# soosiey/gnn-formation-control

Hardware: NVIDIA B200
Metric: agent-graphs/sec fwd+bwd (GSO build+K-hop filter) (higher is better)
Workload: dtype f32

## Files before the change

### gnn-formation-control_b200/csrc/gfc_tc5_wide.cu

```cuda
#include <cuda.h>
#include <cudaTypedefs.h>
#include <type_traits>
#include "gfc_common.cuh"
#include "gfc_tc5.cuh"
#include "gfc_tc5_wide.cuh"
#include <string.h>

namespace gfc {
using tc5::make_desc;
using tc5::store_chunk_f16;

constexpr int kWideTop = 14;
constexpr int kPackHeader = 256;

template <int CIN, int COUT, int NP>
struct WideLayout {
  static constexpr int ROWS = 128;
  static constexpr int CS = CIN / 2;
  static constexpr int CPT = CS / 2;
  static constexpr int NCH = CS / 8;
  static constexpr int PW = ROWS * 16;
  static constexpr int PLANE = NCH * PW;
  static constexpr int SLAB = NP * PLANE;
  static constexpr int STAGE = COUT * 32 * NP;
  static constexpr int KSTEPS = CS / 16;
  static constexpr int PHASE = KSTEPS * STAGE;
  static constexpr int NSTAGE = 2;
  static constexpr int OFF_W = 0;
  static constexpr int OFF_RING = OFF_W + 4 * SLAB;
  static constexpr int OFF_STAGE = (OFF_RING + NSTAGE * PHASE + 1023) / 1024 * 1024;
  static constexpr int OFF_BIAS = OFF_STAGE + ROWS * 128;
  static constexpr int OFF_SP = OFF_BIAS + COUT * 4;
  static constexpr int OFF_DEG = OFF_SP + 2 * ROWS * 8;
  static constexpr int OFF_TAB = OFF_DEG + 2 * 2 * ROWS * 4;
  static constexpr int OFF_MAX = OFF_TAB + 3 * 128 * 4;
  static constexpr int OFF_BAR = OFF_MAX + 64;
  static constexpr int NBAR = 2 * NSTAGE + 2 + 2 + 2 + 1 + 2 + 2 + 2;
  static constexpr int BYTES = OFF_BAR + NBAR * 8 + 16;
  static constexpr int TM_OUT = 0;
  static constexpr int TM_HOP = 2 * COUT;
  static constexpr int TM_P = 2 * COUT + 2 * CS;
  static constexpr int TM_USED = 2 * COUT + 2 * CS + 128;
  static constexpr int TM_COLS = TM_USED <= 32 ? 32 : TM_USED <= 64 ? 64 : TM_USED <= 128 ? 128 : TM_USED <= 256 ? 256 : 512;
  static_assert(CIN % 32 == 0 && CIN >= 32 && CIN <= 128, "CIN in {32,64,96,128}");
  static_assert(COUT % 32 == 0 && COUT >= 32 && COUT <= 128, "COUT multiple of 32, <= 128");
  static_assert(CPT % 8 == 0, "whole chunks per worker thread");
  static_assert(BYTES <= 227 * 1024, "shared memory");
};
__device__ __forceinline__ int row_degree(const int* sdeg, int pbuf, int row) {
  const int* p = sdeg + pbuf * 2 * 128 + row;
  return p[0] + p[128];
}
__device__ __forceinline__ int row_degree4(const int* sdeg, int pbuf, int row) {
  const int* p = sdeg + pbuf * 4 * 128 + row;
  return p[0] + p[128] + p[256] + p[384];
}

constexpr int kWideThreads = 576;
constexpr int kGroupWarps = 8;
int g_wide_flush_every = 3;
int g_wide_no_prefetch = 0;

static __device__ __noinline__ bool wide_adjacent_exact(float ax, float ay, float bx, float by, double thr) {
  return sqdist64(ax, ay, bx, by) <= thr;
}

__device__ __forceinline__ uint32_t adjacency8(const float2* __restrict__ sp, float2 me, int pr, int c0, int c_lo,
                                               int c_hi, int rows_used, double thr, float thr_lo, float thr_hi) {
  const int lo = max(c_lo, c0) - c0, hi = min(min(c_hi, rows_used), c0 + 8) - c0;
  if (hi <= lo || pr >= rows_used) return 0u;
  uint32_t valid = ((1u << hi) - 1u) & ~((1u << lo) - 1u);
  if ((unsigned)(pr - c0) < 8u) valid &= ~(1u << (pr - c0));
  uint32_t in = 0, out = 0;
#pragma unroll
  for (int i = 0; i < 8; ++i) {
    const float2 o = sp[c0 + i];
    const float dx = me.x - o.x, dy = me.y - o.y;
    const float sv = fmaf(dx, dx, dy * dy);
    in |= (sv < thr_lo ? 1u : 0u) << i;
    out |= (sv > thr_hi ? 1u : 0u) << i;
  }
  uint32_t bits = in & valid;
  uint32_t band = valid & ~in & ~out;
  while (band) {
    const int i = __ffs(band) - 1;
    band &= band - 1;
    const float2 o = sp[c0 + i];
    if (wide_adjacent_exact(me.x, me.y, o.x, o.y, thr)) bits |= 1u << i;
  }
  return bits;
}
__device__ __forceinline__ uint32_t dense8(const float* __restrict__ Sg, int N, int transpose, int nr, int pr, int c0,
                                           int c_lo, int c_hi, int rows_used) {
  const int lo = max(c_lo, c0) - c0, hi = min(min(c_hi, rows_used), c0 + 8) - c0;
  if (hi <= lo || pr >= rows_used) return 0u;
  float v[8];
#pragma unroll
  for (int i = 0; i < 8; ++i) {
    const int m = c0 + i - c_lo;
    const bool ok = i >= lo && i < hi;
    const float* p = transpose ? Sg + (size_t)(ok ? m : 0) * N + nr : Sg + (size_t)nr * N + (ok ? m : 0);
    v[i] = ok ? __ldg(p) : 0.f;
  }
  uint32_t bits = 0;
#pragma unroll
  for (int i = 0; i < 8; ++i) bits |= (v[i] != 0.f ? 1u : 0u) << i;
  return bits;
}
__device__ __forceinline__ uint32_t p_word(uint32_t bits, int lo, uint32_t pv) {
  return ((bits >> lo) & 1u) * pv + ((bits >> (lo + 1)) & 1u) * (pv << 16);
}

__device__ __forceinline__ float ldg_f32(const float* p, bool pred) {
  float v;
  asm volatile(
      "{\n\t.reg .pred q;\n\t"
      "setp.ne.b32 q, %2, 0;\n\t"
      "mov.f32 %0, 0f00000000;\n\t"
      "@q ld.global.nc.f32 %0, [%1];\n\t}"
      : "=f"(v)
      : "l"(p), "r"((int)pred));
  return v;
}
__device__ __forceinline__ size_t wide_mask_word(int tile, int gw, int s, int lane) {
  return (((size_t)tile * 8 + gw) * 2 + s) * 32 + lane;
}
__device__ __forceinline__ size_t wide_fmask_word(int tile, int gw, int pcw, int lane) {
  return (((size_t)tile * 8 + gw) * 2 + pcw) * 32 + lane;
}
__device__ __forceinline__ size_t wide_fmask_locate(int tile, int row, int c, int F, int* shift) {
  const int hc = F >> 1, half = c >= hc ? 1 : 0, cc = c - half * hc;
  *shift = cc & 31;
  return wide_fmask_word(tile, half * 4 + (((row >> 5) + 2) & 3), cc >> 5, row & 31);
}
__device__ __forceinline__ uint32_t ldg_u32(const uint32_t* p, bool pred) {
  uint32_t v;
  asm volatile(
      "{\n\t.reg .pred q;\n\t"
      "setp.ne.b32 q, %2, 0;\n\t"
      "mov.b32 %0, 0;\n\t"
      "@q ld.global.nc.b32 %0, [%1];\n\t}"
      : "=r"(v)
      : "l"(p), "r"((int)pred));
  return v;
}
__device__ __forceinline__ float4 ldg_f32x4(const float* p, bool pred) {
  float4 v;
  asm volatile(
      "{\n\t.reg .pred q;\n\t"
      "setp.ne.b32 q, %5, 0;\n\t"
      "mov.f32 %0, 0f00000000;\n\tmov.f32 %1, 0f00000000;\n\tmov.f32 %2, 0f00000000;\n\tmov.f32 %3, 0f00000000;\n\t"
      "@q ld.global.nc.v4.f32 {%0,%1,%2,%3}, [%4];\n\t}"
      : "=f"(v.x), "=f"(v.y), "=f"(v.z), "=f"(v.w)
      : "l"(p), "r"((int)pred));
  return v;
}

__device__ __forceinline__ void red_add_f32(float* p, float v) {
  asm volatile("red.global.add.f32 [%0], %1;" ::"l"(p), "f"(v) : "memory");
}
__device__ __forceinline__ float ldg_cg(const float* p) {
  float v;
  asm volatile("ld.global.cg.f32 %0, [%1];" : "=f"(v) : "l"(p) : "memory");
  return v;
}
__device__ __forceinline__ void group_b_bar() { asm volatile("bar.sync 2, 256;" ::: "memory"); }
__device__ __forceinline__ void group_a_bar() { asm volatile("bar.sync 3, 256;" ::: "memory"); }

struct WideMaps { CUtensorMap m[2]; };

__device__ __forceinline__ float act_fast(float v, float neg, bool use_min) {
  const float t = v * neg;
  return use_min ? fminf(v, t) : fmaxf(v, t);
}

__device__ __forceinline__ void fill_degree_tables(float* tab, int tid, int nthreads) {
  for (int d = tid; d < 128; d += nthreads) {
    const float fd = (float)d;
    tab[d] = d ? 1.f / sqrtf(fd) : 1.f;
    tab[128 + d] = d ? 1.f / fd : 0.f;
    tab[256 + d] = d ? sqrtf(fd) : 1.f;
  }
}

template <int CIN, int COUT, int MODE, int NP>
__global__ void __launch_bounds__(kWideThreads, 1)
tc5_wide_kernel(const __grid_constant__ WideArgs w, const __grid_constant__ WideMaps maps) {
  using L = WideLayout<CIN, COUT, NP>;
  extern __shared__ __align__(128) unsigned char wsmem[];
  unsigned char* Wb = wsmem + L::OFF_W;
  unsigned char* Rb = wsmem + L::OFF_RING;
  float2* sp_all = reinterpret_cast<float2*>(wsmem + L::OFF_SP);
  int* sdeg = reinterpret_cast<int*>(wsmem + L::OFF_DEG);
  float* dtab = reinterpret_cast<float*>(wsmem + L::OFF_TAB);
  uint32_t* smax = reinterpret_cast<uint32_t*>(wsmem + L::OFF_MAX);
  unsigned char* stage_out = wsmem + L::OFF_STAGE;
  float* sbias = reinterpret_cast<float*>(wsmem + L::OFF_BIAS);
  uint64_t* bars = reinterpret_cast<uint64_t*>(wsmem + L::OFF_BAR);
  uint64_t* h_full = bars;
  uint64_t* h_empty = bars + L::NSTAGE;
  uint64_t* w_ready = bars + 2 * L::NSTAGE;
  uint64_t* hop_done = w_ready + 2;
  uint64_t* w0_free = hop_done + 2;
  uint64_t* p_ready = w0_free + 2;
  uint64_t* out_full = p_ready + 1;
  uint64_t* out_free = out_full + 2;
  uint64_t* w0_ready = out_free + 2;
  uint32_t* tmem_ptr = reinterpret_cast<uint32_t*>(w0_ready + 2);

  const int tid = threadIdx.x, lane = tid & 31, warp = tid >> 5;
  const int N = w.N, K = w.K;
  const bool norm = w.g.norm != 0;
  const int tiles_per_cta = (w.ntiles + (int)gridDim.x - 1) / (int)gridDim.x;
  const int t_begin = min(w.ntiles, (int)blockIdx.x * tiles_per_cta);
  const int t_end = min(w.ntiles, t_begin + tiles_per_cta);

  for (int i = tid; i < COUT; i += kWideThreads) sbias[i] = (MODE != 1 && w.bias) ? __ldg(w.bias + i) : 0.f;
  fill_degree_tables(dtab, tid, kWideThreads);
  if (tid == 0) {
    for (int i = 0; i < L::NSTAGE; ++i) { tc5::mbar_init(&h_full[i], 1); tc5::mbar_init(&h_empty[i], 1); }
    for (int i = 0; i < 2; ++i) {
      tc5::mbar_init(&w_ready[i], kGroupWarps);
      tc5::mbar_init(&w0_ready[i], kGroupWarps);
      tc5::mbar_init(&hop_done[i], 1);
      tc5::mbar_init(&w0_free[i], 1);
      tc5::mbar_init(&out_full[i], 1);
      tc5::mbar_init(&out_free[i], kGroupWarps);
    }
    tc5::mbar_init(p_ready, kGroupWarps);
    tc5::fence_mbar_init();
  }
  if (warp == 1) tc5::tmem_alloc(tmem_ptr, L::TM_COLS);
  tc5::fence_proxy_async();
  tc5::fence_before_sync();
  __syncthreads();
  tc5::fence_after_sync();
  const uint32_t tmem = *tmem_ptr;

  if (warp == 0) {
    if (tc5::elect_one()) {
      constexpr uint32_t kIdescTap = tc5::idesc_f16(128, COUT, 0, 0);
      constexpr uint32_t kIdescHop = tc5::idesc_f16(128, L::CS, 0, 1);
      const uint32_t w_addr = tc5::smem_u32(Wb), r_addr = tc5::smem_u32(Rb);
      uint32_t par_wr = 0, par_w0 = 0, par_of = 0, par_pr = 0, par_hf = 0;
      int st = 0;
      const int hop_ksteps = (w.gpc * N + 15) >> 4;
      int it = 0;
      int nstamp = 0;
      const bool dbg = w.dbg != nullptr && blockIdx.x == 0;
#ifdef GFC_WIDE_TIMELINE
#define GFC_WSTAMP(tag) do { if (dbg && nstamp < 2000) { w.dbg[2 * nstamp] = clock64(); w.dbg[2 * nstamp + 1] = (tag); ++nstamp; } } while (0)
#else
#define GFC_WSTAMP(tag) do { (void)dbg; (void)nstamp; } while (0)
#endif
      for (int tile = t_begin; tile < t_end; ++tile, ++it) {
        const int ob = it & 1;
        GFC_WSTAMP(1);
        if (K > 1) { tc5::mbar_wait(p_ready, par_pr); par_pr ^= 1; }
        GFC_WSTAMP(3);
        const uint32_t d_out = tmem + L::TM_OUT + ob * COUT;
#pragma unroll 1
        for (int ph = 0; ph < 2 * K; ++ph) {
          const int k = ph >> 1, s = ph & 1;
          GFC_WSTAMP(100 + ph);
          if (k == 0) { tc5::mbar_wait(&w0_ready[s], (par_w0 >> s) & 1); par_w0 ^= 1u << s; }
          else { tc5::mbar_wait(&w_ready[s], (par_wr >> s) & 1); par_wr ^= 1u << s; }
          tc5::fence_after_sync();
          GFC_WSTAMP(200 + ph);
          const uint32_t ws = w_addr + (2 * s + ((it * K + k) & 1)) * L::SLAB;
          if (k + 1 < K) {
            const uint32_t d_hop = tmem + L::TM_HOP + s * L::CS;
            uint32_t pa = tmem + L::TM_P + ob * 64;
            uint64_t bd = make_desc(ws, 128, L::PW);
            uint32_t acc = 0;
#pragma unroll 1
            for (int j = 0; j < hop_ksteps; ++j) {
              tc5::mma_bf16_ts(d_hop, pa, bd, kIdescHop, acc);
              if (NP == 2) tc5::mma_bf16_ts(d_hop, pa, bd + (L::PLANE >> 4), kIdescHop, 1u);
              acc = 1;
              pa += 8; bd += 256 >> 4;
            }
            tc5::mma_commit(&hop_done[s]);
          }
          if (ph == 0 && it >= 2) { tc5::mbar_wait(&out_free[ob], (par_of >> ob) & 1); par_of ^= 1u << ob; }
          tc5::mbar_wait(&h_full[st], (par_hf >> st) & 1); par_hf ^= 1u << st;
          tc5::fence_after_sync();
          {
            uint64_t a0 = make_desc(ws, L::PW, 128);
            uint64_t b0 = make_desc(r_addr + st * L::PHASE, COUT * 16, 128);
#pragma unroll
            for (int i = 0; i < L::KSTEPS; ++i) {
              tc5::mma_bf16_ss(d_out, a0, b0, kIdescTap, (ph == 0 && i == 0) ? 0u : 1u);
              if (NP == 2) {
                tc5::mma_bf16_ss(d_out, a0, b0 + ((COUT * 32) >> 4), kIdescTap, 1u);
                tc5::mma_bf16_ss(d_out, a0 + (L::PLANE >> 4), b0, kIdescTap, 1u);
              }
              a0 += (2 * L::PW) >> 4; b0 += L::STAGE >> 4;
            }
          }
          tc5::mma_commit(&h_empty[st]);
          st ^= 1;
          if (k == K - 2) tc5::mma_commit(&w0_free[s]);
          GFC_WSTAMP(300 + ph);
        }
        tc5::mma_commit(&out_full[ob]);
      }
#undef GFC_WSTAMP
    }
    __syncwarp();
  } else if (warp == 1) {
    if (tc5::elect_one()) {
      int st = 0;
// ... 281 lines not shown
          asm volatile("prefetch.global.L2 [%0];" ::"l"(yb + off));
      }
      if (tile + 1 < t_end) {
        const int nb = min(w.gpc, w.B - (b0 + w.gpc)) * N * CIN * 4;
        const char* db = reinterpret_cast<const char*>(w.in + (size_t)(b0 + w.gpc) * N * CIN);
        for (int off = wt * 128; off < nb; off += 32 * kGroupWarps * 128)
          asm volatile("prefetch.global.L2 [%0];" ::"l"(db + off));
      }
#pragma unroll 1
      for (int i0 = wt; i0 < n4; i0 += 8 * 32 * kGroupWarps) {
        float4 v[8];
#pragma unroll
        for (int u = 0; u < 8; ++u) {
          const int i = i0 + u * 32 * kGroupWarps;
          v[u] = ldg_f32x4(reinterpret_cast<const float*>(p + (i < n4 ? i : 0)), i < n4);
        }
#pragma unroll
        for (int u = 0; u < 8; ++u)
          m = fmaxf(fmaxf(m, fmaxf(fabsf(v[u].x), fabsf(v[u].y))), fmaxf(fabsf(v[u].z), fabsf(v[u].w)));
      }
      if (MODE == 1 && w.act == GFC_ACT_LEAKY_RELU && w.slope > 1.f) m *= w.slope;
      return m;
    };
    auto epilogue = [&](int tile, int ob, float inv) {
      const int b0 = tile * w.gpc;
      tc5::mbar_wait_suspend(&out_full[ob], (par_ofl >> ob) & 1); par_ofl ^= 1u << ob;
      tc5::fence_after_sync();
      GFC_KSTAMP(500);
      uint32_t fmw = 0;
      static_assert((COUT / 32) % 2 == 0, "two 16-channel pieces per mask word");
#pragma unroll 1
      for (int pc = 0; pc < COUT / 32; ++pc) {
        const int col = half * (COUT / 2) + pc * 16;
        uint32_t v[16];
        tc5::tmem_ld16(tm_lane + L::TM_OUT + ob * COUT + col, v);
        tc5::tmem_ld_wait();
        if constexpr (MODE != 1) {
          float4 o[4];
#pragma unroll
          for (int i4 = 0; i4 < 4; ++i4) {
            const float4 bb = *reinterpret_cast<const float4*>(sbias + col + i4 * 4);
            o[i4].x = act_fast(fmaf(__uint_as_float(v[i4 * 4 + 0]), inv, bb.x), act_neg, act_min);
            o[i4].y = act_fast(fmaf(__uint_as_float(v[i4 * 4 + 1]), inv, bb.y), act_neg, act_min);
            o[i4].z = act_fast(fmaf(__uint_as_float(v[i4 * 4 + 2]), inv, bb.z), act_neg, act_min);
            o[i4].w = act_fast(fmaf(__uint_as_float(v[i4 * 4 + 3]), inv, bb.w), act_neg, act_min);
          }
          if (w.fmask_out) {
            uint32_t b16 = 0;
#pragma unroll
            for (int i4 = 0; i4 < 4; ++i4)
              b16 |= ((o[i4].x > 0.f ? 1u : 0u) | (o[i4].y > 0.f ? 2u : 0u) | (o[i4].z > 0.f ? 4u : 0u) |
                      (o[i4].w > 0.f ? 8u : 0u)) << (4 * i4);
            if (r >= min(w.gpc, w.B - b0) * N) b16 = 0;
            fmw |= b16 << ((pc & 1) * 16);
            if (pc & 1) { w.fmask_out[wide_fmask_word(tile, gw, pc >> 1, lane)] = fmw; fmw = 0; }
          }
          if (lane == 0) tc5::tma_store_wait_read();
          __syncwarp();
          unsigned char* srow = slot_out + lane * 64;
          const int sw = (lane >> 1) & 3;
#pragma unroll
          for (int i4 = 0; i4 < 4; ++i4) *reinterpret_cast<float4*>(srow + ((i4 ^ sw) << 4)) = o[i4];
          tc5::fence_proxy_async();
          __syncwarp();
          if (lane == 0 && hq > 0) {
            tc5::tma_store_2d(my_map, slot_out, col, b0 * N + q * 32);
            tc5::tma_store_commit();
          }
        } else {
          const int rows_used = min(w.gpc, w.B - b0) * N;
          if (r < rows_used) {
            float* dst = w.out + ((size_t)(b0 + jr) * COUT + col) * N + nr;
#pragma unroll
            for (int i = 0; i < 16; ++i) dst[(size_t)i * N] = __uint_as_float(v[i]) * inv;
          }
        }
      }
      tc5::fence_before_sync();
      __syncwarp();
      if (lane == 0) tc5::mbar_arrive(&out_free[ob]);
      GFC_KSTAMP(501);
    };

    int next = t_begin, itn = 0;
    int epi_tile = -1, epi_ob = 0;
    while (true) {
      const bool has_next = next < t_end;
      if (!has_next && epi_tile < 0) break;
      if (has_next) {
        const int pbuf = itn & 1;
        group_b_bar();
        const float m = tile_max(next);
        const uint32_t mw = __reduce_max_sync(0xffffffffu, __float_as_uint(m));
        if (lane == 0) smax[gw] = mw;
        group_b_bar();
        uint32_t mt = smax[0];
#pragma unroll
        for (int i = 1; i < kGroupWarps; ++i) mt = max(mt, smax[i]);
        if (w.amax && wt == 0) atomicMax(reinterpret_cast<unsigned int*>(w.amax) + (MODE == 1 ? 1 : 0), mt);
        if (MODE == 0 && w.mark_stats && w.amax && wt == 0 && blockIdx.x == 0 && itn == 0) w.amax[3] = 1.f;
        scale_next = tc5::pow2_scale(mt, kWideTop, &inv_next);
        rowf_next = 1.f;
        if (norm && K > 1) {
          tc5::mbar_wait_suspend(p_ready, par_pb); par_pb ^= 1;
          tc5::fence_after_sync();
        }
        if (norm) {
          const int d = row_degree(sdeg, pbuf, r);
          rowf_next = dtab[d];
          inv_next *= dtab[256 + d];
        }
        inv_next *= inv_th;
        GFC_KSTAMP(401);
#pragma unroll 1
        for (int s = 0; s < 2; ++s) {
          load_slab(next, s);
          if (itn >= 1 && K >= 2) { tc5::mbar_wait_suspend(&w0_free[s], (par_w0 >> s) & 1); par_w0 ^= 1u << s; }
          GFC_KSTAMP(410 + s);
          store_slab(pbuf, Wb + (2 * s + ((itn * K) & 1)) * L::SLAB);
          tc5::fence_proxy_async();
          tc5::fence_before_sync();
          __syncwarp();
          if (lane == 0) tc5::mbar_arrive(&w0_ready[s]);
          GFC_KSTAMP(420 + s);
        }
      }
      if (epi_tile >= 0) { epilogue(epi_tile, epi_ob, inv_prev); epi_tile = -1; }
      if (has_next) { epi_tile = next; epi_ob = itn & 1; inv_prev = inv_next; ++next; ++itn; }
    }
    if (MODE != 1 && lane == 0) tc5::tma_store_wait_all();
#undef GFC_KSTAMP
  }
  tc5::fence_before_sync();
  __syncthreads();
  if (warp == 1) tc5::tmem_dealloc(tmem, L::TM_COLS);
}

template <int G, int F, int FH, int NP>
struct DhLayout {
  static constexpr int ROWS = 128;
  static constexpr int NFH = F / FH;
  static constexpr int CPT = FH / 4;
  static constexpr int NCH = FH / 8;
  static constexpr int PW = ROWS * 16;
  static constexpr int PLANE = NCH * PW;
  static constexpr int VBUF = NP * PLANE;
  static constexpr int P_BYTES = (ROWS / 8) * PW;
  static constexpr int OFF_V = 0;
  static constexpr int OFF_P = OFF_V + 3 * VBUF;
  static constexpr int OFF_SP = OFF_P + 2 * P_BYTES;
  static constexpr int OFF_DEG = OFF_SP + 2 * ROWS * 8;
  static constexpr int OFF_TAB = OFF_DEG + 2 * 4 * ROWS * 4;
  static constexpr int OFF_DB = OFF_TAB + 3 * 128 * 4;
  static constexpr int OFF_BAR = OFF_DB + FH * 4;
  static constexpr int NBAR = 7;
  static constexpr int BYTES_MIN = OFF_BAR + NBAR * 8 + 16;
  static constexpr int BYTES = BYTES_MIN < 120 * 1024 ? 120 * 1024 : BYTES_MIN;
  static constexpr int TM_X = 0;
  static constexpr int TM_ACC = NP * 64;
  static_assert(FH % 32 == 0 && F % FH == 0 && CPT % 8 == 0, "feature slice");
  static_assert(G == 128 || G == 64 || G == 32, "G");
  static_assert(BYTES <= 227 * 1024, "shared memory");
};

template <int G, int F, int FH, int NP, bool NV4>
__global__ void __launch_bounds__(kWideThreads, 1)
tc5_wide_dh_kernel(const __grid_constant__ WideDhArgs w) {
  using L = DhLayout<G, F, FH, NP>;
  extern __shared__ __align__(128) unsigned char wsmem[];
  unsigned char* Vb = wsmem + L::OFF_V;
  unsigned char* Pb = wsmem + L::OFF_P;
  float2* sp_all = reinterpret_cast<float2*>(wsmem + L::OFF_SP);
  int* sdeg = reinterpret_cast<int*>(wsmem + L::OFF_DEG);
  float* dtab = reinterpret_cast<float*>(wsmem + L::OFF_TAB);
  float* dbs = reinterpret_cast<float*>(wsmem + L::OFF_DB);
  uint64_t* bars = reinterpret_cast<uint64_t*>(wsmem + L::OFF_BAR);
  uint64_t* v_ready = bars;
  uint64_t* hop_done = bars + 1;
  uint64_t* item_done = bars + 2;
  uint64_t* p_ready = bars + 3;
  uint64_t* x_ready = bars + 4;
  uint64_t* v0_ready = bars + 5;
  uint64_t* v0_free = bars + 6;
  uint32_t* tmem_ptr = reinterpret_cast<uint32_t*>(bars + 7);

  const int tid = threadIdx.x, lane = tid & 31, warp = tid >> 5;
  const int N = w.N, K = w.K;
  const bool norm = w.g.norm != 0;
  const int fh = blockIdx.x % L::NFH, part = blockIdx.x / L::NFH, nparts = gridDim.x / L::NFH;
  const int TM_HOP = L::TM_ACC + K * FH;
  const bool merged = NP == 2 && (K + 2) * FH <= 384;
  const int tiles_per_part = (w.ntiles + nparts - 1) / nparts;
  const int t_begin = min(w.ntiles, part * tiles_per_part);
  const int t_end = min(w.ntiles, t_begin + tiles_per_part);

  for (int i = tid; i < 2 * L::P_BYTES / 16; i += kWideThreads) reinterpret_cast<uint4*>(Pb)[i] = make_uint4(0, 0, 0, 0);
  for (int i = tid; i < FH; i += kWideThreads) dbs[i] = 0.f;
  fill_degree_tables(dtab, tid, kWideThreads);
  if (tid == 0) {
    tc5::mbar_init(v_ready, kGroupWarps);
    tc5::mbar_init(hop_done, 1);
    tc5::mbar_init(item_done, 1);
    tc5::mbar_init(p_ready, kGroupWarps);
    tc5::mbar_init(x_ready, kGroupWarps);
    tc5::mbar_init(v0_ready, kGroupWarps);
    tc5::mbar_init(v0_free, 1);
    tc5::fence_mbar_init();
  }
  if (warp == 1) tc5::tmem_alloc(tmem_ptr, 512);
  tc5::fence_proxy_async();
  tc5::fence_before_sync();
  __syncthreads();
  tc5::fence_after_sync();
  const uint32_t tmem = *tmem_ptr;

  auto publish = [&](uint64_t* bar) {
    tc5::fence_proxy_async();
    tc5::fence_before_sync();
    __syncwarp();
    if (lane == 0) tc5::mbar_arrive(bar);
  };

  if (warp == 0) {
    if (tc5::elect_one()) {
      constexpr uint32_t kIdesc = tc5::idesc_f16(128, FH, 0, 1);
      constexpr uint32_t kIdescHop2 = tc5::idesc_f16(128, 2 * FH, 0, 1);
      const uint32_t v_addr = tc5::smem_u32(Vb), p_addr = tc5::smem_u32(Pb);
      uint32_t par_vr = 0, par_v0 = 0, par_pr = 0, par_xr = 0;
      const int ksteps = (w.gpc * N + 15) >> 4;
      int it = 0, vbase = 0;
      int nstamp = 0;
      const bool dbg = w.dbg != nullptr && blockIdx.x == 0;
#ifdef GFC_WIDE_TIMELINE
#define GFC_WSTAMP(tag) do { if (dbg && nstamp < 2000) { w.dbg[2 * nstamp] = clock64(); w.dbg[2 * nstamp + 1] = (tag); ++nstamp; } } while (0)
#else
#define GFC_WSTAMP(tag) do { (void)dbg; (void)nstamp; } while (0)
#endif
      for (int tile = t_begin; tile < t_end; ++tile, ++it) {
        GFC_WSTAMP(1);
        if (K > 1) { tc5::mbar_wait(p_ready, par_pr); par_pr ^= 1; }
        GFC_WSTAMP(3);
        const bool fresh = it == 0 || ((it + part) % w.flush_every) == 0;
        const uint32_t pa = p_addr + (it & 1) * L::P_BYTES;
        auto issue_dh = [&](int kk) {
          if (kk == 0) { tc5::mbar_wait(x_ready, par_xr); par_xr ^= 1; tc5::fence_after_sync(); GFC_WSTAMP(260); }
          const uint32_t vs = v_addr + ((vbase + kk) % 3) * L::VBUF;
          const uint32_t d_acc = tmem + L::TM_ACC + kk * FH;
#pragma unroll 1
          for (int j = 0; j < ksteps; ++j) {
            const uint32_t xa = tmem + L::TM_X + j * 8;
            const uint64_t b0 = make_desc(vs + j * 256, 128, L::PW);
            const uint32_t first = (fresh && j == 0) ? 0u : 1u;
            tc5::mma_bf16_ts(d_acc, xa, b0, kIdesc, first);
            if (NP == 2) {
              const uint64_t b1 = make_desc(vs + L::PLANE + j * 256, 128, L::PW);
              tc5::mma_bf16_ts(d_acc, xa, b1, kIdesc, 1u);
              tc5::mma_bf16_ts(d_acc, xa + 64, b0, kIdesc, 1u);
            }
          }
          if (K >= 3 && kk == K - 3) tc5::mma_commit(v0_free);
          GFC_WSTAMP(300 + kk);
        };
#pragma unroll 1
        for (int k = 0; k < K; ++k) {
          GFC_WSTAMP(100 + k);
          if (k == 0) { tc5::mbar_wait(v0_ready, par_v0); par_v0 ^= 1; }
          else { tc5::mbar_wait(v_ready, par_vr); par_vr ^= 1; }
          tc5::fence_after_sync();
          GFC_WSTAMP(200 + k);
          if (k + 1 < K) {
            const uint32_t vs = v_addr + ((vbase + k) % 3) * L::VBUF;
            uint32_t acc = 0;
#pragma unroll 1
            for (int j = 0; j < ksteps; ++j) {
              const uint64_t da = make_desc(pa + j * 2 * L::PW, L::PW, 128);
              if (merged) {
                tc5::mma_bf16_ss(tmem + TM_HOP, da, make_desc(vs + j * 256, 128, L::PW), kIdescHop2, acc);
                acc = 1;
              } else {
#pragma unroll
                for (int pl = 0; pl < NP; ++pl) {
                  tc5::mma_bf16_ss(tmem + TM_HOP, da, make_desc(vs + pl * L::PLANE + j * 256, 128, L::PW), kIdesc, acc);
                  acc = 1;
                }
              }
            }
            tc5::mma_commit(hop_done);
            GFC_WSTAMP(250 + k);
          }
          if (k >= 1) issue_dh(k - 1);
        }
        issue_dh(K - 1);
        tc5::mma_commit(item_done);
        vbase = (vbase + K) % 3;
      }
#undef GFC_WSTAMP
    }
    __syncwarp();
  } else if (warp >= 2 && warp < 2 + kGroupWarps) {
    const int gw = warp - 2;
    const int wa = tid - 64;
    const int q = warp & 3;
    const int half = gw >> 2;
    const int r = q * 32 + lane;
    const int jr = r / N;
    const uint32_t tm_lane = tmem + ((uint32_t)(q * 32) << 16);
    constexpr int CPA = FH / 2;
    const uint32_t pval = (uint32_t)(15 - w.cshift) << 10;
    float2 mypos = make_float2(0.f, 0.f);
    int degcnt = 0;
    auto load_pos = [&](int tile) {
      const int b0 = tile * w.gpc;
      const int rows_used = min(w.gpc, w.B - b0) * N;
      if (wa < 128 && w.g.pos)
        mypos = (wa < rows_used) ? __ldg(reinterpret_cast<const float2*>(w.g.pos) + (size_t)b0 * N + wa) : make_float2(0.f, 0.f);
    };
    auto build_p_part = [&](int tile, int pbuf, int t0, int t1) {
      const float2* sp = sp_all + pbuf * L::ROWS;
      unsigned char* pb = Pb + pbuf * L::P_BYTES;
      const int rows_used = min(w.gpc, w.B - tile * w.gpc) * N;
      const int c_lo = jr * N, c_hi = c_lo + N;
      const float2 me = sp[r];
      if (r < w.gpc * N) {
#pragma unroll 1
        for (int t = t0; t < t1; ++t) {
          const int qc = 2 * t + half;
          if (qc * 8 < c_hi && qc * 8 + 8 > c_lo) {
            const uint32_t bits =
                w.g.S ? dense8(w.g.S + (size_t)(tile * w.gpc + jr) * w.g.s_bstride, N, w.g.s_transpose, r - c_lo, r, qc * 8,
                               c_lo, c_hi, rows_used)
                      : adjacency8(sp, me, r, qc * 8, c_lo, c_hi, rows_used, w.g.thr, w.g.thr_lo, w.g.thr_hi);
            degcnt += __popc(bits);
            *reinterpret_cast<uint4*>(pb + qc * L::PW + r * 16) =
                make_uint4(p_word(bits, 0, pval), p_word(bits, 2, pval), p_word(bits, 4, pval), p_word(bits, 6, pval));
          }
        }
      }
    };
    auto publish_p = [&](int pbuf) {
      sdeg[(pbuf * 2 + half) * L::ROWS + r] = degcnt;
      degcnt = 0;
      publish(p_ready);
    };
    const int nslots = K - 1;
    const int cps = nslots ? (8 + nslots - 1) / nslots : 8;
    if (K > 1 && t_begin < t_end) {
      load_pos(t_begin);
      if (wa < 128) sp_all[wa] = mypos;
      group_a_bar();
      if (t_begin + 1 < t_end) load_pos(t_begin + 1);
      build_p_part(t_begin, 0, 0, 8);
      publish_p(0);
    }
    uint32_t par_hd = 0;
    int vbase = 0, it = 0;
    int nstamp = 0;
    const bool dbg = w.dbg != nullptr && blockIdx.x == 0 && tid == 64;
#ifdef GFC_WIDE_TIMELINE
#define GFC_KSTAMP(tag) do { if (dbg && nstamp < 2000) { w.dbg[4096 + 2 * nstamp] = clock64(); w.dbg[4096 + 2 * nstamp + 1] = (tag); ++nstamp; } } while (0)
#else
#define GFC_KSTAMP(tag) do { (void)dbg; (void)nstamp; } while (0)
#endif
    for (int tile = t_begin; tile < t_end; ++tile, ++it) {
      float wbf = 1.f;
      const bool has_next = K > 1 && tile + 1 < t_end;
      const int pbn = (it + 1) & 1;
      if (K > 1) {
        if (has_next && wa < 128) sp_all[pbn * L::ROWS + wa] = mypos;
        group_a_bar();
        if (tile + 2 < t_end) load_pos(tile + 2);
      }
#pragma unroll 1
      for (int k = 0; k + 1 < K; ++k) {
        GFC_KSTAMP(100 + k);
        tc5::mbar_wait_suspend(hop_done, par_hd); par_hd ^= 1;
        tc5::fence_after_sync();
        GFC_KSTAMP(200 + k);
        if (norm && k == 0) wbf = dtab[128 + row_degree(sdeg, it & 1, r)];
        unsigned char* base = Vb + ((vbase + k + 1) % 3) * L::VBUF + (half * (CPA / 8)) * L::PW + r * 16;
        const uint32_t taddr = tm_lane + TM_HOP + half * CPA;
#pragma unroll
        for (int hh = 0; hh < CPA / 16; ++hh) {
          uint32_t v[16], v2[16];
          tc5::tmem_ld16(taddr + hh * 16, v);
          if (merged) tc5::tmem_ld16(taddr + FH + hh * 16, v2);
          tc5::tmem_ld_wait();
#pragma unroll
          for (int c = 0; c < 2; ++c) {
            float f[8];
#pragma unroll
            for (int i = 0; i < 8; ++i) {
              float t = __uint_as_float(v[c * 8 + i]);
              if (merged) t += __uint_as_float(v2[c * 8 + i]);
              f[i] = norm ? t * wbf : t;
            }
            store_chunk_f16<NP>(base + (hh * 2 + c) * L::PW, L::PLANE, f);
          }
        }
// ... 89 lines not shown
          for (int rho = 0; rho < 2; ++rho) {
#pragma unroll
            for (int i = 0; i < 4; ++i) {
              float f0 = s_x;
              if (norm) f0 *= dtab[256 + row_degree(sdeg, pbuf, qtr * 32 + 16 * rho + 4 * (lane & 3) + i)];
              rf[rho][i] = f0;
            }
          }
#pragma unroll
          for (int h16 = 0; h16 < 2; ++h16) {
            uint32_t p0[8], p1[8];
#pragma unroll
            for (int rho = 0; rho < 2; ++rho) {
#pragma unroll
              for (int gs = 0; gs < 2; ++gs) {
                const float* src = &xt[16 * h16 + 8 * rho + 4 * gs];
                const float a = src[0] * rf[rho][0], b = src[1] * rf[rho][1], c = src[2] * rf[rho][2], d = src[3] * rf[rho][3];
                if (NP == 2) {
                  tc5::split_f16x2(a, b, p0[4 * rho + 2 * gs], p1[4 * rho + 2 * gs]);
                  tc5::split_f16x2(c, d, p0[4 * rho + 2 * gs + 1], p1[4 * rho + 2 * gs + 1]);
                } else {
                  p0[4 * rho + 2 * gs] = tc5::pack_f16x2(a, b);
                  p0[4 * rho + 2 * gs + 1] = tc5::pack_f16x2(c, d);
                }
              }
            }
            const uint32_t ta = tmem + ((uint32_t)(q * 32 + 16 * h16) << 16) + L::TM_X + qtr * 16;
            tc5::tmem_st_16x256b_x2(ta, p0);
            if (NP == 2) tc5::tmem_st_16x256b_x2(ta + 64, p1);
          }
        }
        if (qq == 1) tc5::tmem_st_wait();
      }
      if (qq == 1) {
        tc5::fence_before_sync();
        __syncwarp();
        if (lane == 0) tc5::mbar_arrive(x_ready);
      }
    };
    auto load_v0 = [&](int tile) {
      const int b0 = tile * w.gpc;
      const int rows_used = min(w.gpc, w.B - b0) * N;
      const bool bits = w.dpre == nullptr && w.vmask != nullptr && w.act != GFC_ACT_NONE;
      const bool masked = w.dpre == nullptr && !bits && w.act != GFC_ACT_NONE;
      const float* src = w.dpre ? w.dpre : w.dY;
      if (w.fmask != nullptr && w.act != GFC_ACT_NONE) {
        const bool relu = w.act == GFC_ACT_RELU;
        const int c = fh * FH + 4 * (lane % PPR);
        int sh_unused = 0;
        const int wc_l = (lane >> 4) < FH / 32 ? (lane >> 4) : 0;
        const uint32_t myword =
            ldg_u32(w.fmask + wide_fmask_locate(tile, 16 * gw + (lane & 15), fh * FH + 32 * wc_l, F, &sh_unused), true);
#pragma unroll
        for (int i = 0; i < NPC; ++i) {
          const int row = 16 * gw + RPI * i + lane / PPR;
          const float4 v = ldg_f32x4(w.dY + ((size_t)b0 * N + row) * F + c, row < rows_used);
          xin[4 * i] = v.x; xin[4 * i + 1] = v.y; xin[4 * i + 2] = v.z; xin[4 * i + 3] = v.w;
        }
        const int wc = (4 * (lane % PPR)) >> 5, sh = (4 * (lane % PPR)) & 31;
#pragma unroll
        for (int i = 0; i < NPC; ++i) {
          const uint32_t nib = __shfl_sync(0xffffffffu, myword, wc * 16 + RPI * i + lane / PPR) >> sh;
#pragma unroll
          for (int e = 0; e < 4; ++e)
            xin[4 * i + e] = ((nib >> e) & 1u) ? xin[4 * i + e] : relu ? 0.f : __fmul_rn(xin[4 * i + e], w.slope);
        }
        return;
      }
      if (bits) {
        const bool relu = w.act == GFC_ACT_RELU;
        constexpr int PPRX = F / 8, RPIX = 32 / PPRX;
        constexpr bool same_map = (2 * FH == F);
        uint32_t mw[same_map ? 1 : NPC];
#pragma unroll
        for (int i = 0; i < NPC; ++i) {
          const int ro = RPI * i + lane / PPR;
          const int row = 16 * gw + ro;
          const bool ok = row < rows_used;
          const size_t off = ((size_t)b0 * N + row) * F + fh * FH + 4 * (lane % PPR);
          const float4 v = ldg_f32x4(src + off, ok);
          xin[4 * i] = v.x; xin[4 * i + 1] = v.y; xin[4 * i + 2] = v.z; xin[4 * i + 3] = v.w;
          if (same_map) {
            if (i == 0) mw[0] = ldg_u32(w.vmask + wide_mask_word(tile, gw, fh, lane), true);
          } else {
            const int q = (fh * FH) / 4 + lane % PPR;
            mw[i] = ldg_u32(w.vmask + wide_mask_word(tile, gw, q / PPRX, (ro % RPIX) * PPRX + q % PPRX), true);
          }
        }
#pragma unroll
        for (int i = 0; i < NPC; ++i) {
          const int ro = RPI * i + lane / PPR;
          const uint32_t nib = same_map ? (mw[0] >> (4 * i)) : (mw[same_map ? 0 : i] >> (4 * (ro / RPIX)));
#pragma unroll
          for (int e = 0; e < 4; ++e)
            xin[4 * i + e] = ((nib >> e) & 1u) ? xin[4 * i + e] : relu ? 0.f : __fmul_rn(xin[4 * i + e], w.slope);
        }
        return;
      }
#pragma unroll
      for (int hb = 0; hb < NPC; hb += 4) {
        float4 vv[4], yy[4];
        size_t off[4];
        bool ok[4];
#pragma unroll
        for (int i = 0; i < 4; ++i) {
          const int row = 16 * gw + RPI * (hb + i) + lane / PPR;
          ok[i] = row < rows_used;
          off[i] = ((size_t)b0 * N + row) * F + fh * FH + 4 * (lane % PPR);
          vv[i] = ldg_f32x4(src + off[i], ok[i]);
        }
        if (masked) {
#pragma unroll
          for (int i = 0; i < 4; ++i) yy[i] = ldg_f32x4(w.yout + off[i], ok[i]);
#pragma unroll
          for (int i = 0; i < 4; ++i) {
            vv[i].x = act_grad(vv[i].x, yy[i].x, w.act, w.slope);
            vv[i].y = act_grad(vv[i].y, yy[i].y, w.act, w.slope);
            vv[i].z = act_grad(vv[i].z, yy[i].z, w.act, w.slope);
            vv[i].w = act_grad(vv[i].w, yy[i].w, w.act, w.slope);
          }
        }
#pragma unroll
        for (int i = 0; i < 4; ++i) {
          xin[4 * (hb + i)] = vv[i].x; xin[4 * (hb + i) + 1] = vv[i].y; xin[4 * (hb + i) + 2] = vv[i].z; xin[4 * (hb + i) + 3] = vv[i].w;
        }
      }
    };
    auto store_v0 = [&](unsigned char* vbuf, int pbuf) {
      const int pi = lane % PPR;
      const bool odd = pi & 1;
#pragma unroll
      for (int i = 0; i < NPC; ++i) {
        dbacc[0] += xin[4 * i]; dbacc[1] += xin[4 * i + 1]; dbacc[2] += xin[4 * i + 2]; dbacc[3] += xin[4 * i + 3];
      }
#pragma unroll
      for (int i = 0; i < NPC; i += 2) {
        float snd[4], rcv[4], own[4];
#pragma unroll
        for (int e = 0; e < 4; ++e) {
          snd[e] = odd ? xin[4 * i + e] : xin[4 * (i + 1) + e];
          own[e] = odd ? xin[4 * (i + 1) + e] : xin[4 * i + e];
        }
#pragma unroll
        for (int e = 0; e < 4; ++e) rcv[e] = __shfl_xor_sync(0xffffffffu, snd[e], 1);
        const int row = 16 * gw + RPI * (i + (odd ? 1 : 0)) + lane / PPR;
        float f0 = s_v;
        if (norm) f0 *= dtab[row_degree(sdeg, pbuf, row)];
        float v[8];
#pragma unroll
        for (int e = 0; e < 4; ++e) { v[e] = (odd ? rcv[e] : own[e]) * f0; v[4 + e] = (odd ? own[e] : rcv[e]) * f0; }
        store_chunk_f16<NP>(vbuf + (pi >> 1) * L::PW + row * 16, L::PLANE, v);
      }
    };
    float* dst = w.dHp + (size_t)part * F * K * G;
    auto flush = [&]() {
      tc5::fence_after_sync();
      if (q * 32 < G) {
        float unscale = inv_sx * inv_sv;
        const float up = __uint_as_float((uint32_t)(127 + w.cshift) << 23);
#pragma unroll 1
        for (int k = 0; k < K; ++k) {
#pragma unroll 1
          for (int cb = 0; cb < FH / 2; cb += 8) {
            const int col = half * (FH / 2) + cb;
            uint32_t v[8];
            tc5::tmem_ld8u(tm_lane + L::TM_ACC + k * FH + col, v);
            tc5::tmem_ld_wait();
            if (g_ok) {
              float* d0 = dst + (size_t)(fh * FH + col) * K * G + k * G + r;
#pragma unroll
              for (int i = 0; i < 8; ++i) red_add_f32(d0 + (size_t)i * K * G, __uint_as_float(v[i]) * unscale);
            }
          }
          unscale *= up;
        }
      }
      tc5::fence_before_sync();
    };

    int vbase_next = 0, n_items = 0, itn = 0;
    for (int next = t_begin; next < t_end; ++next, ++itn) {
      const int pbuf = itn & 1;
      if (wt == 0 && w.no_prefetch == 2) {
        if (itn == 0) prefetch_tile(next);
        if (next + 1 < t_end) prefetch_tile(next + 1);
      }
      load_v0(next);
      if (norm && K > 1) {
        tc5::mbar_wait_suspend(p_ready, par_pb); par_pb ^= 1;
        tc5::fence_after_sync();
      }
      if (itn >= 1 && K >= 3) { tc5::mbar_wait_suspend(v0_free, par_vf); par_vf ^= 1; }
      GFC_KSTAMP(410);
      store_v0(Vb + (vbase_next % 3) * L::VBUF, pbuf);
      publish(v0_ready);
      GFC_KSTAMP(420);
      load_xt(next, 0);
      if (itn >= 1) {
        GFC_KSTAMP(500);
        tc5::mbar_wait_suspend(item_done, par_id); par_id ^= 1;
        GFC_KSTAMP(501);
        ++n_items;
        if (((n_items + part) % w.flush_every) == 0) flush();
        GFC_KSTAMP(502);
      }
      store_xt(pbuf, 0);
      load_xt(next, 1);
      store_xt(pbuf, 1);
      GFC_KSTAMP(510);
      vbase_next = (vbase_next + K) % 3;
    }
    if (itn >= 1) {
      tc5::mbar_wait_suspend(item_done, par_id); par_id ^= 1;
      flush();
    }
#undef GFC_KSTAMP
    if (w.dbp) {
#pragma unroll
      for (int i = 0; i < 4; ++i) atomicAdd(dbs + 4 * (lane % PPR) + i, dbacc[i]);
      group_b_bar();
      if (wt < FH) w.dbp[(size_t)part * F + fh * FH + wt] = dbs[wt];
    }
  }
  tc5::fence_before_sync();
  __syncthreads();
  if (warp == 1) tc5::tmem_dealloc(tmem, 512);
}

__global__ void __launch_bounds__(1024)
wide_pack_taps_kernel(const float* __restrict__ h, int G, int F, int K, int mode, int cshift, int planes,
                      unsigned char* __restrict__ outb) {
  __shared__ uint32_t swmax[32];
  const int total = K * G * F;
  float m = 0.f;
  {
    const float4* h4 = reinterpret_cast<const float4*>(h);
    const int n4 = total >> 2;
    for (int i0 = threadIdx.x; i0 < n4; i0 += 8 * 1024) {
      float4 v[8];
#pragma unroll
      for (int u = 0; u < 8; ++u) {
        const int i = i0 + u * 1024;
        v[u] = i < n4 ? __ldg(h4 + i) : make_float4(0.f, 0.f, 0.f, 0.f);
      }
#pragma unroll
      for (int u = 0; u < 8; ++u) m = fmaxf(fmaxf(m, fmaxf(fabsf(v[u].x), fabsf(v[u].y))), fmaxf(fabsf(v[u].z), fabsf(v[u].w)));
    }
  }
  const uint32_t mw = __reduce_max_sync(0xffffffffu, __float_as_uint(m));
  if ((threadIdx.x & 31) == 0) swmax[threadIdx.x >> 5] = mw;
  __syncthreads();
  uint32_t mt = swmax[0];
  for (int i = 1; i < 32; ++i) mt = max(mt, swmax[i]);
  float inv_th;
  int top = kWideTop - cshift * (K - 1);
  if (top < -8) top = -8;
  const float t_h = tc5::pow2_scale(mt, top, &inv_th);
  if (blockIdx.x == 0 && threadIdx.x == 0) reinterpret_cast<float*>(outb)[0] = inv_th;
  uint16_t* out = reinterpret_cast<uint16_t*>(outb + kPackHeader);
  const int CIN = mode == 0 ? G : F, COUT = mode == 0 ? F : G;
  for (int idx = blockIdx.x * blockDim.x + threadIdx.x; idx < total; idx += gridDim.x * blockDim.x) {
    const int f = idx / (K * G), rem = idx - f * K * G;
    const int k = rem / G, g = rem - k * G;
    const int ch = mode == 0 ? g : f, n = mode == 0 ? f : g;
    const float v = __ldg(h + idx) * t_h * __uint_as_float((uint32_t)(127 + cshift * k) << 23);
    const __half hi = __float2half_rn(v);
    const int c16 = ch >> 4, cc = (ch >> 3) & 1, e = ch & 7;
    const size_t stage = (size_t)(k * (CIN / 16) + c16) * (COUT * 16 * planes);
    const size_t o = stage + (size_t)cc * COUT * 8 + (size_t)n * 8 + e;
    out[o] = __half_as_ushort(hi);
    if (planes == 2) out[o + (size_t)COUT * 16] = __half_as_ushort(__float2half_rn(v - __half2float(hi)));
  }
}

int launch_wide_pack(const float* h, int G, int F, int K, int mode, int cshift, int planes, unsigned char* out,
                     cudaStream_t st) {
  const int total = K * G * F;
  GFC_REQUIRE((reinterpret_cast<uintptr_t>(h) & 15) == 0, GFC_ERR_UNSUPPORTED, "launch_wide_pack: taps must be 16-byte aligned");
  int grid = ceil_div(total, 1024);
  if (grid > 148) grid = 148;
  wide_pack_taps_kernel<<<grid, 1024, 0, st>>>(h, G, F, K, mode, cshift, planes, out);
  GFC_LAUNCH_CHECK("wide_pack_taps_kernel");
  return GFC_OK;
}

__global__ void __launch_bounds__(512)
wide_absmax_kernel(const float* __restrict__ a, size_t n_a, const float* __restrict__ b, size_t n_b, float bscale,
                   float* __restrict__ amax, const float* __restrict__ stats) {
  const size_t stride = (size_t)gridDim.x * blockDim.x * 4;
  const size_t i0 = ((size_t)blockIdx.x * blockDim.x + threadIdx.x) * 4;
  const bool have_a = stats != nullptr && ldg_cg(stats + 3) != 0.f;
  if (have_a && a && blockIdx.x == 0 && threadIdx.x == 0)
    atomicMax(reinterpret_cast<unsigned int*>(amax), __float_as_uint(ldg_cg(stats)));
  for (int which = 0; which < 2; ++which) {
    const float* p = which ? b : a;
    const size_t n = which ? n_b : n_a;
    if (!p || (which == 0 && have_a)) continue;
    float m = 0.f;
    const bool vec = (reinterpret_cast<uintptr_t>(p) & 15) == 0;
    for (size_t i = i0; i < n; i += stride) {
      if (vec && i + 4 <= n) {
        const float4 v = __ldg(reinterpret_cast<const float4*>(p + i));
        m = fmaxf(fmaxf(m, fmaxf(fabsf(v.x), fabsf(v.y))), fmaxf(fabsf(v.z), fabsf(v.w)));
      } else {
        for (size_t j = i; j < n && j < i + 4; ++j) m = fmaxf(m, fabsf(__ldg(p + j)));
      }
    }
    if (which) m *= bscale;
    const uint32_t mw = __reduce_max_sync(0xffffffffu, __float_as_uint(m));
    if ((threadIdx.x & 31) == 0 && mw) atomicMax(reinterpret_cast<unsigned int*>(amax) + which, mw);
  }
}

__global__ void wide_stats_mark_kernel(float* stats) { stats[3] = 1.f; }
int launch_stats_mark(float* stats, cudaStream_t st) {
  wide_stats_mark_kernel<<<1, 1, 0, st>>>(stats);
  GFC_LAUNCH_CHECK("wide_stats_mark_kernel");
  return GFC_OK;
}

int launch_wide_absmax(const float* a, size_t n_a, const float* b, size_t n_b, float bscale, float* amax,
                       const float* stats, cudaStream_t st) {
  if (!a && !b) return GFC_OK;
  DeviceInfo di;
  int rc = get_device_info(&di);
  if (rc) return rc;
  const size_t n = n_a > n_b ? n_a : n_b;
  size_t want = (n + 2047) / 2048;
  int grid = (int)(want < (size_t)di.sm_count * 4 ? (want ? want : 1) : (size_t)di.sm_count * 4);
  wide_absmax_kernel<<<grid, 512, 0, st>>>(a, n_a, b, n_b, bscale, amax, stats);
  GFC_LAUNCH_CHECK("wide_absmax_kernel");
  return GFC_OK;
}

size_t wide_mask_bytes(int B, int N) {
  if (B < 1 || N < 1 || N > 128) return 0;
  int gpc = 128 / N; if (gpc > B) gpc = B;
  return (size_t)ceil_div(B, gpc) * 2048;
}

int wide_cshift(int N, int norm) {
  if (norm) return 0;
  int c = 0;
  while ((1 << c) < N - 1) ++c;
  return c;
}

bool wide_supported(int N, int G, int F, int K, int mode) {
  const int CIN = mode == 0 ? G : F, COUT = mode == 0 ? F : G;
  if (N < 1 || N > 128 || K < 1 || K > 16) return false;
  if (wide_cshift(N, 0) * (K - 1) > 21) return false;
  return (CIN == 128 || CIN == 64) && (COUT == 128 || COUT == 64);
}

size_t wide_pack_bytes(int G, int F, int K) { return align_up((size_t)kPackHeader + (size_t)K * G * F * 4, 256); }

static int encode_tmap_2d(CUtensorMap* tm, const void* base, uint64_t inner, uint64_t outer, uint32_t box_inner,
                          uint32_t box_outer, CUtensorMapSwizzle swz) {
  static PFN_cuTensorMapEncodeTiled_v12000 fn = nullptr;
  if (!fn) {
    void* p = nullptr;
    cudaDriverEntryPointQueryResult qres;
// ... 130 lines not shown
```

Measured before the change: 8.181 million.

## Vectorize dH flush via smem staging and overlap drain with per-hop acc barriers

The flush of TMEM accumulators now loads a whole column half per hop, stages it through a per-warp shared-memory transpose, and issues 128-bit vector red.add atomics with coalesced addresses instead of scalar strided atomics. New per-hop acc_free mbarriers let the MMA issuer start the next accumulation into a hop slot as soon as that slot has been read out, rather than implicitly serialising. The flush is moved after the x-tile stores so the stores overlap with the MMA. This adds shared memory and barrier complexity, and carries a risk of ordering bugs around TMEM reuse.

```diff
diff --git a/gnn-formation-control_b200/csrc/gfc_tc5_wide.cu b/gnn-formation-control_b200/csrc/gfc_tc5_wide.cu
--- a/gnn-formation-control_b200/csrc/gfc_tc5_wide.cu
+++ b/gnn-formation-control_b200/csrc/gfc_tc5_wide.cu
@@ -156,8 +156,8 @@
   return v;
 }
 
-__device__ __forceinline__ void red_add_f32(float* p, float v) {
-  asm volatile("red.global.add.f32 [%0], %1;" ::"l"(p), "f"(v) : "memory");
+__device__ __forceinline__ void red_add_f32x4(float* p, float4 v) {
+  asm volatile("red.global.add.v4.f32 [%0], {%1, %2, %3, %4};" ::"l"(p), "f"(v.x), "f"(v.y), "f"(v.z), "f"(v.w) : "memory");
 }
 __device__ __forceinline__ float ldg_cg(const float* p) {
   float v;
@@ -745,8 +745,10 @@
   static constexpr int OFF_DEG = OFF_SP + 2 * ROWS * 8;
   static constexpr int OFF_TAB = OFF_DEG + 2 * 4 * ROWS * 4;
   static constexpr int OFF_DB = OFF_TAB + 3 * 128 * 4;
-  static constexpr int OFF_BAR = OFF_DB + FH * 4;
-  static constexpr int NBAR = 7;
+  static constexpr int OFF_STG = (OFF_DB + FH * 4 + 15) / 16 * 16;
+  static constexpr int OFF_BAR = OFF_STG + 8 * 32 * 32 * 4;
+  static constexpr int KMAX = 384 / FH - 1;
+  static constexpr int NBAR = 7 + KMAX;
   static constexpr int BYTES_MIN = OFF_BAR + NBAR * 8 + 16;
   static constexpr int BYTES = BYTES_MIN < 120 * 1024 ? 120 * 1024 : BYTES_MIN;
   static constexpr int TM_X = 0;
@@ -775,7 +777,9 @@
   uint64_t* x_ready = bars + 4;
   uint64_t* v0_ready = bars + 5;
   uint64_t* v0_free = bars + 6;
-  uint32_t* tmem_ptr = reinterpret_cast<uint32_t*>(bars + 7);
+  uint64_t* acc_free = bars + 7;
+  uint32_t* tmem_ptr = reinterpret_cast<uint32_t*>(bars + L::NBAR);
+  float* stg = reinterpret_cast<float*>(wsmem + L::OFF_STG);
 
   const int tid = threadIdx.x, lane = tid & 31, warp = tid >> 5;
   const int N = w.N, K = w.K;
@@ -798,6 +802,7 @@
     tc5::mbar_init(x_ready, kGroupWarps);
     tc5::mbar_init(v0_ready, kGroupWarps);
     tc5::mbar_init(v0_free, 1);
+    for (int k = 0; k < L::KMAX; ++k) tc5::mbar_init(&acc_free[k], kGroupWarps);
     tc5::fence_mbar_init();
   }
   if (warp == 1) tc5::tmem_alloc(tmem_ptr, 512);
@@ -819,7 +824,7 @@
       constexpr uint32_t kIdesc = tc5::idesc_f16(128, FH, 0, 1);
       constexpr uint32_t kIdescHop2 = tc5::idesc_f16(128, 2 * FH, 0, 1);
       const uint32_t v_addr = tc5::smem_u32(Vb), p_addr = tc5::smem_u32(Pb);
-      uint32_t par_vr = 0, par_v0 = 0, par_pr = 0, par_xr = 0;
+      uint32_t par_vr = 0, par_v0 = 0, par_pr = 0, par_xr = 0, par_af = 0;
       const int ksteps = (w.gpc * N + 15) >> 4;
       int it = 0, vbase = 0;
       int nstamp = 0;
@@ -834,9 +839,12 @@
         if (K > 1) { tc5::mbar_wait(p_ready, par_pr); par_pr ^= 1; }
         GFC_WSTAMP(3);
         const bool fresh = it == 0 || ((it + part) % w.flush_every) == 0;
+        const bool drained = fresh && it > 0;
         const uint32_t pa = p_addr + (it & 1) * L::P_BYTES;
         auto issue_dh = [&](int kk) {
-          if (kk == 0) { tc5::mbar_wait(x_ready, par_xr); par_xr ^= 1; tc5::fence_after_sync(); GFC_WSTAMP(260); }
+          if (kk == 0) { tc5::mbar_wait(x_ready, par_xr); par_xr ^= 1; GFC_WSTAMP(260); }
+          if (drained) { tc5::mbar_wait(&acc_free[kk], (par_af >> kk) & 1); par_af ^= 1u << kk; GFC_WSTAMP(270 + kk); }
+          if (kk == 0 || drained) tc5::fence_after_sync();
           const uint32_t vs = v_addr + ((vbase + kk) % 3) * L::VBUF;
           const uint32_t d_acc = tmem + L::TM_ACC + kk * FH;
 #pragma unroll 1
@@ -1232,30 +1240,39 @@
         store_chunk_f16<NP>(vbuf + (pi >> 1) * L::PW + row * 16, L::PLANE, v);
       }
     };
-    float* dst = w.dHp + (size_t)part * F * K * G;
     auto flush = [&]() {
+      float* dst = w.dHp + (size_t)part * F * K * G;
       tc5::fence_after_sync();
-      if (q * 32 < G) {
-        float unscale = inv_sx * inv_sv;
-        const float up = __uint_as_float((uint32_t)(127 + w.cshift) << 23);
+      float unscale = inv_sx * inv_sv;
+      const float up = __uint_as_float((uint32_t)(127 + w.cshift) << 23);
 #pragma unroll 1
-        for (int k = 0; k < K; ++k) {
-#pragma unroll 1
-          for (int cb = 0; cb < FH / 2; cb += 8) {
-            const int col = half * (FH / 2) + cb;
-            uint32_t v[8];
-            tc5::tmem_ld8u(tm_lane + L::TM_ACC + k * FH + col, v);
-            tc5::tmem_ld_wait();
-            if (g_ok) {
-              float* d0 = dst + (size_t)(fh * FH + col) * K * G + k * G + r;
-#pragma unroll
-              for (int i = 0; i < 8; ++i) red_add_f32(d0 + (size_t)i * K * G, __uint_as_float(v[i]) * unscale);
-            }
-          }
-          unscale *= up;
-        }
-      }
-      tc5::fence_before_sync();
+      for (int k = 0; k < K; ++k) {
+        constexpr int DC = FH / 2;
+        const int col = half * DC;
+        uint32_t v[DC];
+        if (g_ok) {
+          if constexpr (DC == 16) tc5::tmem_ld16(tm_lane + L::TM_ACC + k * FH + col, v);
+          else tc5::tmem_ld32(tm_lane + L::TM_ACC + k * FH + col, v);
+          tc5::tmem_ld_wait();
+        }
+        tc5::fence_before_sync();
+        __syncwarp();
+        if (lane == 0) tc5::mbar_arrive(&acc_free[k]);
+        if (g_ok) {
+          float* sw = stg + gw * 32 * 32;
+#pragma unroll
+          for (int c = 0; c < DC; ++c) sw[c * 32 + lane] = __uint_as_float(v[c]) * unscale;
+          __syncwarp();
+#pragma unroll
+          for (int rd = 0; rd < DC / 4; ++rd) {
+            const int c = rd * 4 + (lane >> 3), j = lane & 7;
+            const float4 t4 = *reinterpret_cast<const float4*>(sw + c * 32 + 4 * j);
+            red_add_f32x4(dst + (size_t)(fh * FH + col + c) * K * G + k * G + q * 32 + 4 * j, t4);
+          }
+          __syncwarp();
+        }
+        unscale *= up;
+      }
     };
 
     int vbase_next = 0, n_items = 0, itn = 0;
@@ -1280,14 +1297,15 @@
         GFC_KSTAMP(500);
         tc5::mbar_wait_suspend(item_done, par_id); par_id ^= 1;
         GFC_KSTAMP(501);
-        ++n_items;
-        if (((n_items + part) % w.flush_every) == 0) flush();
-        GFC_KSTAMP(502);
       }
       store_xt(pbuf, 0);
       load_xt(next, 1);
       store_xt(pbuf, 1);
       GFC_KSTAMP(510);
+      if (itn >= 1 && ((++n_items + part) % w.flush_every) == 0) {
+        flush();
+        GFC_KSTAMP(502);
+      }
       vbase_next = (vbase_next + K) % 3;
     }
     if (itn >= 1) {
```

Result: faster. 8.277 million (median of 6 runs) (+1.2%).
